# zeyadmohamedabdo/Visual-Question-Answering-VQA-system

Measured on AMD Instinct MI355X. Metric: image-question pairs/sec (train step), higher is better.
Workload: dtype bf16; 1 GPU; VQA train step fwd+CE+bwd+allreduce+clip+AdamW, batch 512/GPU, 3x224x224 images, 20 tokens, d=256, 4 text layers, 49 image tokens, 1000 answers, dropout on (BASELINE configs[2]); batch_per_gpu=512, global_batch=512, parallelism=dp1, reducer=off

## Files before the change

### include/vqa_hip.h

```cpp
#ifndef VQA_HIP_H
#define VQA_HIP_H
#include <stdint.h>
#ifdef __cplusplus
extern "C" {
#endif
typedef struct ihipStream_t* hipStream_t;

int vqa_igemm_mtiles(int M, int N, int loader);
int vqa_igemm_variant(int dtype, int loader, int M, int N, int Kw, int B, int H, int W, int C, int Ho, int Wo,
                      int R, int S, int stride, int pad);
int vqa_igemm(int dtype, int loader, const void* a, const void* w, void* out, const float* bias, const void* addend,
              const void* addmask, const void* outmask , float* stats, int M, int N, int Kw, int B, int H, int W, int C, int Ho, int Wo,
              int R, int S, int stride, int pad, int transposed, int relu, float drop_p, unsigned long long drop_seed,
              int stats_mode ,
              hipStream_t stream);
int vqa_linear_dgrad_act(int dtype, const void* dz, const void* wt, void* dx, const void* addend, const void* outact, float drop_p,
                         int M, int Kin, int N, hipStream_t stream);
int vqa_wgrad_plan(int dtype, int loader, int M, int N, int Kw, int B, int H, int W, int C, int R, int S, long long* ws_floats,
                   int* kind, int* tile_n, int* tile_k, int* nsplit);
int vqa_wgrad(int dtype, int loader, const void* dy, const void* x, float* dw, int M, int N, int Kw, int B, int H, int W,
              int C, int Ho, int Wo, int R, int S, int stride, int pad, float* ws, long long ws_floats, hipStream_t stream);
int vqa_pack_rows(int dtype, const float* in, void* out, int N, int K, int Kp, hipStream_t stream);
int vqa_pack_transpose(int dtype, const float* in, void* out, int N, int T, int C, int ldo, int col0, int flip, hipStream_t stream);
int vqa_pack_transpose_batch(int dtype, const float* flat, void* out, const long long* desc, int nd, int total_blocks, hipStream_t stream);
// ... 28 lines not shown
                        float* ws , long long ws_floats, hipStream_t stream);
int vqa_wgrad3x3_c128_blocks(int B, int H, int W);
int vqa_wgrad3x3_c128(const void* x, const void* dy, float* dw, int B, int H, int W, float* ws, long long ws_floats, hipStream_t stream);
int vqa_wgrad3x3_c64_blocks(int B, int H, int W);
int vqa_wgrad3x3_c64(const void* x, const void* dy, float* dw , int B, int H, int W,
                     float* ws ,
                     long long ws_floats, hipStream_t stream);
long long vqa_wgrad_group_ws(int dtype, int njobs, const int* M, const int* N, const int* Kw);
int vqa_wgrad_group(int dtype, int njobs, const void* const* dy, const void* const* x, float* const* dw, const int* M, const int* N,
                    const int* Kw, float* ws, long long ws_floats, hipStream_t stream);
int vqa_slab_reduce(const float* ws, float* dw, int nslabs, long long n, hipStream_t stream);
int vqa_dgrad_s2(int dtype, const void* dy, const void* dyd, const void* wt, void* out, int B, int H, int W, int C,
                 int Ho, int Wo, int N, int R, int pad, hipStream_t stream);
int vqa_stem_conv_blocks(int B, int H, int W);
int vqa_stem_pack(const float* w_krsc, void* wstem, hipStream_t stream);
int vqa_stem_conv(const float* img, const void* wstem, void* out, float* stats, int B, int H, int W, hipStream_t stream);
int vqa_stem_conv_pool_ok(int B, int H, int W);
int vqa_stem_conv_pool(const float* img, const void* wstem, const float* coef, void* out, int B, int H, int W, hipStream_t stream);
int vqa_stem_wgrad_blocks(int B, int H, int W);
int vqa_stem_wgrad(const float* img, const void* dy, float* dw , int B, int H, int W,
                   float* ws , long long ws_floats, hipStream_t stream);
int vqa_stem_wgrad_fused(const float* img, const void* y, const void* dpool, const uint8_t* idx, const float* coef,
                         const float* bcoef, float* dw, int B, int H, int W, float* ws, long long ws_floats, hipStream_t stream);
int vqa_stem_dgrad_pack(int dtype, const float* w_krsc, void* wpk, hipStream_t stream);
int vqa_stem_dgrad(int dtype, const void* dy, const void* wpk, float* dimg, int B, int H, int W, hipStream_t stream);
int vqa_stem_dgrad_fused_ok(int B, int H, int W);
int vqa_stem_dgrad_fused(const void* y, const void* dpool, const uint8_t* idx, const float* coef, const float* bcoef, const void* wpk,
                         float* dimg, int B, int H, int W, hipStream_t stream);

int vqa_bn_stats_finalize(const float* part, int tiles, int C, double count, const float* gamma, const float* beta,
                          float* running_mean, float* running_var, long long* num_batches_tracked, float momentum, float eps,
                          double* scratch , float* coef, hipStream_t stream);
int vqa_bn_eval_coef(int C, const float* gamma, const float* beta, const float* running_mean, const float* running_var,
                     float eps, float* coef, hipStream_t stream);
int vqa_bn_apply(int dtype, const void* y, const float* coef, const void* res, const float* rcoef, void* out,
                 long long numel, int C, int relu, hipStream_t stream);
int vqa_bn_apply_pool_chunks(int dtype, int HW, int C);
int vqa_bn_apply_pool(int dtype, const void* y, const float* coef, const void* res, const float* rcoef, void* out, int B, int HW, int C,
// ... 151 lines not shown
```

### visual-question-answering-vqa-system_amd/_lib.py

```python
from __future__ import annotations

import ctypes as C
import os

import torch

_HERE = os.path.dirname(os.path.abspath(__file__))
LIB_PATH = os.path.join(_HERE, "libvqa_hip.so")

P, I, F, D, LL, ULL = C.c_void_p, C.c_int, C.c_float, C.c_double, C.c_longlong, C.c_ulonglong

SIGNATURES = {
    "vqa_gemm8p": [P, P, P, I, I, I, P],
    "vqa_gemm4w": [P, P, P, I, I, I, P],
    "vqa_conv8p_ok": [I, I, I, I, I],
    "vqa_conv8p": [P, P, P, P, P, P, P, P, P, P, I, P, P, I, I, I, I, I, I, I, P],
    "vqa_igemm_mtiles": [I, I, I],
    "vqa_igemm_variant": [I] * 15,
    "vqa_igemm": [I, I, P, P, P, P, P, P, P, P] + [I] * 15 + [F, ULL, I, P],
    "vqa_linear_dgrad_act": [I, P, P, P, P, P, F, I, I, I, P],
    "vqa_wgrad_plan": [I] * 11 + [P, P, P, P, P],
    "vqa_wgrad": [I, I, P, P, P] + [I] * 13 + [P, LL, P],
    "vqa_pack_rows": [I, P, P, I, I, I, P],
    "vqa_pack_transpose": [I, P, P, I, I, I, I, I, I, P],
# ... 7 lines not shown
    "vqa_conv3x3_c64p_epi": [P, P, P, P, P, P, I, I, I, P],
    "vqa_conv3x3_c64p_bnred": [P, P, P, P, P, P, I, I, I, P],
    "vqa_conv3x3_c64p_bn": [P, P, P, P, P, P, P, P, P, P, P, I, I, I, I, D, F, F, P],
    "vqa_wgrad3x3_c64_bn_ok": [I, I, I],
    "vqa_wgrad3x3_c64_bn": [P, P, P, P, I, I, I, P, LL, P],
    "vqa_wgrad3x3_c128_blocks": [I, I, I],
    "vqa_wgrad3x3_c128": [P, P, P, I, I, I, P, LL, P],
    "vqa_wgrad3x3_c64_blocks": [I, I, I],
    "vqa_wgrad3x3_c64": [P, P, P, I, I, I, P, LL, P],
    "vqa_wgrad_group_ws": [I, I, P, P, P],
    "vqa_wgrad_group": [I, I, P, P, P, P, P, P, P, LL, P],
    "vqa_slab_reduce": [P, P, I, LL, P],
    "vqa_dgrad_s2": [I, P, P, P, P, I, I, I, I, I, I, I, I, I, P],
    "vqa_stem_conv_blocks": [I, I, I],
    "vqa_stem_pack": [P, P, P],
    "vqa_stem_conv": [P, P, P, P, I, I, I, P],
    "vqa_stem_conv_pool_ok": [I, I, I],
    "vqa_stem_conv_pool": [P, P, P, P, I, I, I, P],
    "vqa_stem_wgrad_blocks": [I, I, I],
    "vqa_stem_wgrad": [P, P, P, I, I, I, P, LL, P],
    "vqa_stem_wgrad_fused": [P, P, P, P, P, P, P, I, I, I, P, LL, P],
    "vqa_stem_dgrad_pack": [I, P, P, P],
    "vqa_stem_dgrad": [I, P, P, P, I, I, I, P],
    "vqa_stem_dgrad_fused_ok": [I, I, I],
    "vqa_stem_dgrad_fused": [P, P, P, P, P, P, P, I, I, I, P],
    "vqa_bn_stats_finalize": [P, I, I, D, P, P, P, P, P, F, F, P, P, P],
    "vqa_bn_eval_coef": [I, P, P, P, P, F, P, P],
    "vqa_bn_apply": [I, P, P, P, P, P, LL, I, I, P],
    "vqa_bn_apply_pool_chunks": [I, I, I],
    "vqa_bn_apply_pool": [I, P, P, P, P, P, I, I, I, I, P, P],
    "vqa_se_bwd_blocks": [I, I, I, I],
    "vqa_se_bwd_scratch": [I, I, I, I, I],
    "vqa_bn_bwd_blocks": [LL],
    "vqa_bn_bwd_reduce": [I, P, P, P, P, P, P, P, LL, I, I, I, P],
    "vqa_bn_acc_words": [I, I],
    "vqa_bn_apply_acc": [I, P, P, P, P, P, P, P, P, P, P, P, P, P, P, P, P, P, I, I, I, I, D, F, F, P, P],
# ... 45 lines not shown
    "vqa_answer_scores": [P, P, P, P, I, I, I, I, P, P],
    "vqa_cross_entropy_soft": [I, P, P, P, I, P, P, P, I, I, F, P, P, P, P, P],
    "vqa_challenge_accuracy_update": [P, P, P, I, P, I, I, P],
    "vqa_convert": [I, I, P, P, LL, P],
    "vqa_sumsq": [P, LL, P, P],
    "vqa_image_normalize": [P, P, P, I, I, I, F, F, F, F, F, F, P],
    "vqa_image_color_jitter": [P, P, P, I, I, I, P, P, F, F, F, F, F, F, P, P],
    "vqa_image_resize_ws": [I, P, P, I, I, I],
    "vqa_image_resize": [P, P, P, P, P, I, I, I, I, I, P, P, P, F, F, F, F, F, F, P, LL, P],
    "vqa_pack_tokens": [P, P, P, P, I, I, I, I, I, I, P],
    "vqa_adamw": [P, P, P, P, LL, F, F, F, F, F, LL, P, F, F, P, P, P, P],
    "vqa_sumsq_ranges": [P, P, I, LL, P, P],
    "vqa_adamw_ranges": [P, P, P, P, P, I, LL, F, F, F, F, F, LL, P, F, F, P, P, P, P, I, P, P],
}
_RET_LL = {"vqa_image_resize_ws", "vqa_wgrad_group_ws", "vqa_spatial_bwd_scratch", "vqa_se_bwd_scratch", "vqa_layernorm_bwd_ws", "vqa_bias_act_bwd_ws"}
_NO_STATUS = _RET_LL | {"vqa_wgrad3x3_c64_blocks", "vqa_bn_acc_words", "vqa_bn_apply_pool_chunks", "vqa_se_bwd_blocks", "vqa_wgrad3x3_c128_blocks", "vqa_layernorm_bwd_folds", "vqa_bias_act_bwd_fold_rows", "vqa_conv3x3_c64p_blocks", "vqa_stem_wgrad_blocks", "vqa_igemm_mtiles", "vqa_igemm_variant", "vqa_bn_bwd_blocks", "vqa_stem_conv_blocks", "vqa_stem_conv_pool_ok", "vqa_stem_dgrad_fused_ok", "vqa_wgrad3x3_c64_bn_ok", "vqa_conv8p_ok"}

_lib = None


def lib() -> C.CDLL:
    global _lib
    if _lib is None:
        if not os.path.exists(LIB_PATH):
            raise RuntimeError(f"{LIB_PATH} is missing: build it with __graft_entry__.build() "
                               "(hipcc --offload-arch=gfx950); there is no CPU fallback")
        L = C.CDLL(LIB_PATH)
        for name, args in SIGNATURES.items():
            fn = getattr(L, name)
            fn.argtypes = args
            fn.restype = LL if name in _RET_LL else I
# ... 39 lines not shown
```

### visual-question-answering-vqa-system_amd/csrc/stem_conv.hip

```cpp
#include <cstdlib>
#include "common.h"
#include <type_traits>
#include "stem_route.h"

namespace {
constexpr int RB = 4;
constexpr int PR = 2 * RB + 5;
constexpr int KP = 192;
constexpr int LDW = KP + 8;
constexpr int LDCS = 64 + 8;
}

template <int PROWS, int XO, int CH>
__device__ __forceinline__ void stem_fill_patch(bf16_t* __restrict__ patch, int PW, __amdgpu_buffer_rsrc_t rsImg, int b, int ih_base,
                                                int H, int W, int tid) {
  static_assert(XO & 1, "odd column offset");
  const int W4 = W >> 2, nitems = 3 * PROWS * W4, nh = PW - W;
  const float inv_w4 = 1.0f / (float)W4, inv_nh = 1.0f / (float)nh;
  for (int i = tid; i < 3 * PROWS * nh; i += 256) {
    const int row = (int)(((float)i + 0.5f) * inv_nh), k = i - row * nh;
    patch[row * PW + (k < XO ? k : W + k)] = 0;
  }
  for (int base = tid; base < nitems; base += 256 * CH) {
    f32x4 v[CH]; int dst[CH];
#pragma unroll
// ... 18 lines not shown
      d[3] = f2bf(v[i][3]);
    }
  }
}

__global__ void stem_pack_kernel(const float* __restrict__ w, bf16_t* __restrict__ out) {
  const int i = blockIdx.x * blockDim.x + threadIdx.x;
  if (i >= 64 * KP) return;
  const int n = i / KP, k = i - n * KP, pair = k >> 3, s = k & 7;
  float v = 0.f;
  if (pair < 21 && s < 7) { const int c = pair / 7, r = pair - c * 7; v = w[((n * 7 + r) * 7 + s) * 3 + c]; }
  out[i] = f2bf(v);
}

__global__ __launch_bounds__(256) void stem_conv_kernel(const float* __restrict__ img, const bf16_t* __restrict__ wst, bf16_t* __restrict__ out,
                                                        float* __restrict__ stats, int H, int W, int Ho, int Wo) {
  extern __shared__ __attribute__((aligned(16))) char smem[];
  const int PW = 2 * Wo + 8;
  bf16_t* patch = reinterpret_cast<bf16_t*>(smem);
  bf16_t* Wl = patch + 3 * PR * PW;
  bf16_t* Cst = Wl;
  float* red = reinterpret_cast<float*>(Wl + 64 * LDW);
  const int tid = threadIdx.x, lane = tid & 63, wave = tid >> 6, g = lane >> 4, li = lane & 15;
  const int rblocks = Ho / RB;
  const int b = blockIdx.x / rblocks, oh0 = (blockIdx.x - b * rblocks) * RB;

  for (int v = tid; v < 64 * (KP / 8); v += 256) {
    const int n = v / (KP / 8), kv = v - n * (KP / 8);
    *reinterpret_cast<u32x4*>(&Wl[n * LDW + kv * 8]) = *reinterpret_cast<const u32x4*>(&wst[n * KP + kv * 8]);
  }
  const int ih_base = 2 * oh0 - 3;
// ... 2 lines not shown
    const int iw = x - 3;
    const bool cok = iw >= 0 && iw < W;
    float vals[3 * PR];
#pragma unroll
    for (int row = 0; row < 3 * PR; ++row) {
      const int c = row / PR, pr = row - c * PR, ih = ih_base + pr;
      const bool ok = cok && ih >= 0 && ih < H;
      const int ihc = min(max(ih, 0), H - 1), iwc = min(max(iw, 0), W - 1);
      const float t = __builtin_bit_cast(float, __builtin_amdgcn_raw_buffer_load_b32(rsImg, (((b * 3 + c) * H + ihc) * W + iwc) * 4, 0, 0));
      vals[row] = ok ? t : 0.f;
    }
#pragma unroll
    for (int row = 0; row < 3 * PR; ++row) patch[row * PW + x] = f2bf(vals[row]);
  }
  __syncthreads();

  bf16x8 bfr[6][4];
#pragma unroll
  for (int kk = 0; kk < 6; ++kk)
#pragma unroll
    for (int nt = 0; nt < 4; ++nt)
      bfr[kk][nt] = *reinterpret_cast<const bf16x8*>(&Wl[(nt * 16 + li) * LDW + kk * 32 + g * 8]);
  __syncthreads();

  float ssum[4] = {0.f, 0.f, 0.f, 0.f}, ssq[4] = {0.f, 0.f, 0.f, 0.f};
  const int mtiles_row = Wo / 16, mtiles = RB * mtiles_row;
  bf16_t* mycs = Cst + wave * 16 * LDCS;
  for (int mt = wave; mt < mtiles; mt += 4) {
    const int orow = mt / mtiles_row, ow0 = (mt - orow * mtiles_row) * 16;
    f32x4 acc[4];
// ... 310 lines not shown
  for (int j = 0; j < 3; ++j) {
    const int k2 = wave * 48 + j * 16 + li, pair = k2 >> 3, s = k2 & 7;
    if (pair >= 21 || s >= 7) continue;
    const int c = pair / 7, r = pair - c * 7;
#pragma unroll
    for (int i = 0; i < 4; ++i)
#pragma unroll
      for (int rr = 0; rr < 4; ++rr) {
        const size_t o = (size_t)(i * 16 + g * 4 + rr) * 147 + (r * 7 + s) * 3 + c;
        if (ws) ws[(size_t)blockIdx.x * (64 * 147) + o] = acc[i][j][rr];
        else atomicAdd(dw + o, acc[i][j][rr]);
      }
  }
}

extern "C" int vqa_slab_reduce(const float* ws, float* dw, int nslabs, long long n, hipStream_t st);

static size_t stem_wgrad_shm(int Wo, int nsplit) {
  const int PW = 2 * Wo + 8, MP = (Wo / nsplit + 31) / 32 * 32;
  return (size_t)(3 * PRW * PW + MP * LDA + MP * LDD) * 2;
}
static int stem_nsplit(int Wo) {
  const int env = vqa_env_int("VQA_STEM_NSPLIT", 0);
  if (env > 0 && Wo % (8 * env) == 0) return env;
  const int floor_ = Wo > 64 ? 2 : 1;
  for (int n = floor_; n <= 16; ++n)
    if (Wo % (8 * n) == 0 && stem_wgrad_shm(Wo, n) <= (size_t)160 * 1024 / 3) return n;
  return floor_;
}
static int stem_wgrad_grid(int B, int Ho, int Wo, size_t* shm_out) {
  const size_t shm = stem_wgrad_shm(Wo, stem_nsplit(Wo));
  if (shm_out) *shm_out = shm;
  if (shm > 160 * 1024) return 0;
  const int nblocks = B * (Ho / RBW);
  const int cap = 256 * (int)((160 * 1024) / shm > 4 ? 4 : (160 * 1024) / shm);
  return nblocks < cap ? nblocks : cap;
}

extern "C" {

int vqa_stem_conv_blocks(int B, int H, int W) {
  const int Ho = (H + 6 - 7) / 2 + 1, Wo = (W + 6 - 7) / 2 + 1;
  if (Ho % RB || Wo % 16 || Wo > 256) return 0;
  return B * (Ho / RB);
}
int vqa_stem_pack(const float* w_krsc, void* wstem , hipStream_t st) {
  if (!w_krsc || !wstem) return VQA_EARG;
  hipLaunchKernelGGL(stem_pack_kernel, dim3((64 * KP + 255) / 256), dim3(256), 0, st, w_krsc, (bf16_t*)wstem);
  VQA_LAUNCH_CHECK(); return VQA_OK;
}
int vqa_stem_conv(const float* img, const void* wstem, void* out, float* stats, int B, int H, int W, hipStream_t st) {
  const int nb = vqa_stem_conv_blocks(B, H, W);
  if (!img || !wstem || !out || nb <= 0 || (size_t)B * 3 * H * W * 4 >= 0x7fffffffull) return VQA_EARG;
  const int Ho = (H + 6 - 7) / 2 + 1, Wo = (W + 6 - 7) / 2 + 1, PW = 2 * Wo + 8;
  const size_t shm = (size_t)(3 * PR * PW + 64 * LDW) * 2 + 4 * 64 * 2 * 4;
  (void)vqa_ensure_lds(reinterpret_cast<const void*>(&stem_conv_kernel), shm);
  hipLaunchKernelGGL(stem_conv_kernel, dim3(nb), dim3(256), shm, st, img, (const bf16_t*)wstem, (bf16_t*)out, stats, H, W, Ho, Wo);
  VQA_LAUNCH_CHECK(); return VQA_OK;
}

static size_t stem_conv_pool_shm(int H, int W, int* ctiles_out, int* pw_out) {
  const int Ho = (H + 6 - 7) / 2 + 1, Wo = (W + 6 - 7) / 2 + 1, Hp = (Ho + 2 - 3) / 2 + 1, Wp = (Wo + 2 - 3) / 2 + 1;
  if (H < 7 || W < 7 || (Ho & 1) || (Wo & 1) || Hp % PRB) return 0;
  const int ctiles = (Wp + 6) / 7;
  const int PW = (2 * (14 * ctiles + 2) + 8 + 7) / 8 * 8;
  if (ctiles_out) *ctiles_out = ctiles;
  if (pw_out) *pw_out = PW;
  const size_t shm = (size_t)(3 * PRP * PW + 64 * LDW) * 2;
  return shm <= 160 * 1024 ? shm : 0;
}
int vqa_stem_conv_pool_ok(int B, int H, int W) {
  return B > 0 && stem_conv_pool_shm(H, W, nullptr, nullptr) > 0 && (size_t)B * 3 * H * W * 4 < 0x7fffffffull;
// ... 41 lines not shown
  const int nsplit = stem_nsplit(Wo);
  const int PW = 2 * Wo + 8, MP = (Wo / nsplit + 31) / 32 * 32;
  const size_t shm = (size_t)(3 * PRW * PW + MP * LDA + MP * LDD) * 2;
  if (shm > 160 * 1024) return VQA_EARG;
  (void)vqa_ensure_lds(reinterpret_cast<const void*>(&stem_wgrad_kernel<true>), shm);
  int nblocks = B * (Ho / RBW);
  const int cap = 256 * (int)((160 * 1024) / shm > 4 ? 4 : (160 * 1024) / shm);
  int grid = nblocks < cap ? nblocks : cap;
  float* w = (ws && ws_floats >= (long long)grid * 64 * 147) ? ws : nullptr;
  hipLaunchKernelGGL(stem_wgrad_kernel<true>, dim3(grid), dim3(256), shm, st, img, (const bf16_t*)y, dw, B, H, W, Ho, Wo,
                     (const bf16_t*)dpool, idx, coef, bcoef, Hp, Wp, nsplit, w);
  VQA_LAUNCH_CHECK();
  return w ? vqa_slab_reduce(w, dw, grid, 64 * 147, st) : VQA_OK;
}

}
```

### visual-question-answering-vqa-system_amd/engine.py

```python
from __future__ import annotations

import math
from typing import Callable, Dict, List, Optional

import torch

from . import kernels as K
from . import layout as LY
from ._lib import call, dt, ptr


def _streams_overlap(a: "torch.cuda.Stream", b: "torch.cuda.Stream", cycles: int = 1_500_000) -> bool:
    ea, eb = torch.cuda.Event(), torch.cuda.Event()
    with torch.cuda.stream(a):
        torch.cuda._sleep(cycles)
        ea.record()
    with torch.cuda.stream(b):
        torch.cuda._sleep(1000)
        eb.record()
    eb.synchronize()
    ok = not ea.query()
    ea.synchronize()
    return ok

# ... 55 lines not shown
        self.fuse_bn1_reduce = True
        self.use_conv8p_bwd = True
        self._accbuf = None
        self._accpos = 0
        self._stem_fcoef = None
        self.fold_eval = True
        self._fold = None
        self.infer_precision = "bf16"
        self._foldmx = None
        self.stem_w = None
        self.side, self.side2 = pick_concurrent_streams(flat.device, 2) if flat.is_cuda else (None, None)
        self.two_streams = True
        self.capture = None
        self.capture_io = None
        self.fuse_stem_eval = True
        self.mark = None

    def P(self, name):
        e = self.E[name]
        return self.flat[e.offset: e.offset + e.numel]

    def Wm(self, name):
        return LY.mat_of(self.wsrc, self.E[name])

    def _packT(self, key, pieces, rows, ld):
        t = self._wt.get(key)
        if t is None:
            t = torch.empty((rows, ld), device=self.flat.device, dtype=self.dtype)
            for off, n, tt, c, col0, flip in pieces:
                K.pack_transpose(self.flat[off: off + n * tt * c].view(n, tt, c), self.dtype, out=t, ldo=ld, col0=col0, flip=flip)
# ... 369 lines not shown
        phead = cfg["answer_dropout"] if htrain else 0.0
        dev = images.device

        main = torch.cuda.current_stream()
        use_side = self.two_streams and self.side is not None
        if use_side:
            ev0 = torch.cuda.Event(); ev0.record(main)
        H1, W1 = (IH + 6 - 7) // 2 + 1, (IW + 6 - 7) // 2 + 1
        M = B * H1 * W1
        sgeom = (B, IH, IW, 3, H1, W1, 7, 7, 2, 3)
        Hp, Wp = (H1 + 2 - 3) // 2 + 1, (W1 + 2 - 3) // 2 + 1
        x = None
        if self.fuse_stem_eval and not training and not cnn_tape and self.stem_w2 is not None:
            x = K.stem_conv_pool(images, self.stem_w2, self._bn_coef("image_encoder.stem.1", None, 0, 64, M, False), B, IH, IW)
        if x is None:
            if self.stem_w2 is not None and K.stem_conv_blocks(B, IH, IW) > 0:
                y, st, mt = K.stem_conv(images, self.stem_w2, B, IH, IW, training)
            else:
                y, st, mt = K.igemm(images, self.stem_w, M, 64, self.stem_kp, sgeom, dtype=T, loader=K.LOADER_STEM, want_stats=training)
            coef = self._bn_coef("image_encoder.stem.1", st, mt, 64, M, training)
            x = torch.empty((B * Hp * Wp, 64), device=dev, dtype=T)
            idx = torch.empty((B * Hp * Wp, 64), device=dev, dtype=torch.uint8)
            call("vqa_stem_pool_fwd", dt(T), ptr(y), ptr(coef), ptr(x), ptr(idx), B, H1, W1, 64)
            if cnn_tape:
                tape["stem"] = dict(images=images, y=y, coef=coef, idx=idx, geom=sgeom, H1=H1, W1=W1)
        H, W, C = Hp, Wp, 64
        d, heads = cfg["embed_dim"], cfg["num_attention_heads"]
        hd = d // heads
        Bt, L = token_ids.shape
        rows = Bt * L
        pe = self.buf["text_encoder.positional_encoding.pe"]
        if L > pe.shape[1]:
            raise RuntimeError(f"sequence length {L} exceeds max_question_length {pe.shape[1]}")
        text = {}

        def issue_text():
            if use_side:
                self.side.wait_event(ev0)
            with torch.cuda.stream(self.side if use_side else main):
                emb_e = self.E["text_encoder.token_embedding.weight"]
# ... 908 lines not shown
        bc = torch.empty((3, 64), device=dxc.device, dtype=torch.float32)
        bnp = "image_encoder.stem.1"
        call("vqa_bn_bwd_finalize", ptr(slab), nb, 64, 1, float(B * H1 * W1), ptr(self.P(bnp + ".weight")), ptr(st["coef"]),
             int(training), ptr(self._gslice(G, bnp + ".weight")), ptr(self._gslice(G, bnp + ".bias")), ptr(bc))
        if after_reduce is not None:
            after_reduce()
        wpk = K.stem_dgrad_pack(self.P("image_encoder.stem.0.weight"), T) if want_dimg else None
        dimg = None
        skip_w = self._frozen_g(self._gslice(G, "image_encoder.stem.0.weight"))
        if fused and skip_w:
            pass
        elif fused:
            dwv = self._gslice(G, "image_encoder.stem.0.weight")
            e0 = K.prof_begin()
            ws, wsf = K.stem_wgrad_scratch(dxc.device, B, IH, IW)
            call("vqa_stem_wgrad_fused", ptr(st["images"]), ptr(st["y"]), ptr(dxc), ptr(st["idx"]), ptr(st["coef"]), ptr(bc), ptr(dwv), B, IH, IW,
                 ptr(ws), wsf)
            if e0 is not None:
                K.prof_end(e0, "stem_wgrad_kernel<true>", 2.0 * B * H1 * W1 * 64 * 147,
                           B * 3 * IH * IW * 4 + B * H1 * W1 * 64 * 2 + dxc.numel() * 3)
        if fused:
            if want_dimg:
                if K.stem_dgrad_fused_ok(B, IH, IW):
                    dimg = K.stem_dgrad_fused(st["y"], dxc, st["idx"], st["coef"], bc, wpk, B, IH, IW)
                else:
                    dy = torch.empty_like(st["y"])
                    call("vqa_stem_bwd_apply", dt(T), ptr(dxc), ptr(st["idx"]), ptr(st["y"]), ptr(st["coef"]), ptr(bc), ptr(dy), B, H1, W1, 64)
                    dimg = K.stem_dgrad(dy, wpk, B, IH, IW)
        else:
            dy = torch.empty_like(st["y"])
            call("vqa_stem_bwd_apply", dt(T), ptr(dxc), ptr(st["idx"]), ptr(st["y"]), ptr(st["coef"]), ptr(bc), ptr(dy), B, H1, W1, 64)
            if not skip_w:
                K.wgrad(dy, st["images"], LY.mat_of(G, self.E["image_encoder.stem.0.weight"]), B * H1 * W1, 64, 147, st["geom"], dtype=T,
                        loader=K.LOADER_STEM)
            if want_dimg:
# ... 86 lines not shown
```

### visual-question-answering-vqa-system_amd/kernels.py

```python
from __future__ import annotations

import os

import torch

from . import _lib as L
from ._lib import call, dt, ptr

LOADER_NHWC, LOADER_STEM = 0, 1

PROFILE = None
PROFILE_VARIANTS = []
PROFILE_STAGED = {}


def prof_begin():
    if PROFILE is None:
        return None
    e0 = torch.cuda.Event(enable_timing=True)
    e0.record()
    return e0


def prof_end(e0, sym, flops, nbytes):
# ... 270 lines not shown

def stem_dgrad_fused(y, dpool, idx, coef, bc, wpk, B, H, W):
    dimg = torch.empty((B, 3, H, W), device=y.device, dtype=torch.float32)
    Ho, Wo, flops = _stem_dgrad_cost(B, H, W)
    e0 = prof_begin()
    call("vqa_stem_dgrad_fused", ptr(y), ptr(dpool), ptr(idx), ptr(coef), ptr(bc), ptr(wpk), ptr(dimg), B, H, W)
    if e0 is not None:
        prof_end(e0, "stem_dgrad_kernel<bf16,true>", flops, B * Ho * Wo * 64 * 2 + dpool.numel() * 3 + dimg.numel() * 4)
    return dimg


def stem_conv_blocks(B, H, W) -> int:
    return L.count("vqa_stem_conv_blocks", B, H, W)


def stem_conv(img, wstem, B, H, W, want_stats):
    nb = stem_conv_blocks(B, H, W)
    Ho, Wo = (H + 6 - 7) // 2 + 1, (W + 6 - 7) // 2 + 1
    y = torch.empty((B * Ho * Wo, 64), device=img.device, dtype=torch.bfloat16)
    stats = torch.empty((nb, 2, 64), device=img.device, dtype=torch.float32) if want_stats else None
    e0 = prof_begin()
    call("vqa_stem_conv", ptr(img), ptr(wstem), ptr(y), ptr(stats), B, H, W)
    if e0 is not None:
        prof_end(e0, "stem_conv_kernel", 2.0 * B * Ho * Wo * 64 * 147, B * 3 * H * W * 4 + B * Ho * Wo * 64 * 2)
    return y, stats, nb


def stem_conv_pool(img, wstem, coef, B, H, W):
    if not L.count("vqa_stem_conv_pool_ok", B, H, W):
        return None
    Ho, Wo = (H + 6 - 7) // 2 + 1, (W + 6 - 7) // 2 + 1
    Hp, Wp = (Ho + 2 - 3) // 2 + 1, (Wo + 2 - 3) // 2 + 1
    x = torch.empty((B * Hp * Wp, 64), device=img.device, dtype=torch.bfloat16)
    e0 = prof_begin()
    call("vqa_stem_conv_pool", ptr(img), ptr(wstem), ptr(coef), ptr(x), B, H, W)
    if e0 is not None:
        prof_end(e0, "stem_conv_pool_kernel", 2.0 * B * Ho * Wo * 64 * 147, B * 3 * H * W * 4 + B * Hp * Wp * 64 * 2)
    return x

# ... 262 lines not shown
```

### visual-question-answering-vqa-system_amd/layout.py

```python
from __future__ import annotations

import math
from dataclasses import dataclass
from typing import Dict, List, Tuple

import torch

STAGE_CHANNELS = (64, 128, 256, 512)
ALIGN = 8

CONFIG_KEYS = ("vocab_size", "embed_dim", "num_answers", "use_se_attention", "use_spatial_attention", "se_reduction",
               "num_transformer_layers", "num_attention_heads", "ffn_hidden_dim", "max_question_length",
               "num_cross_layers", "use_gating", "dropout", "answer_dropout")


@dataclass
class Entry:
    name: str
    shape: Tuple[int, ...]
    kind: str
    is_param: bool
    offset: int = -1
    krsc: bool = False

# ... 140 lines not shown
def bucket_ranges(entries: List[Entry]) -> List[Tuple[str, int, int]]:
    groups = ["answer_head.", "fusion.", "text_encoder.", "image_encoder.stage4.", "image_encoder.stage3.",
              "image_encoder.stage2.", "image_encoder.stage1.", "image_encoder.stem."]
    out = []
    total = flat_size(entries)
    params = [e for e in entries if e.is_param]
    for g in groups:
        es = [e for e in params if e.name.startswith(g)]
        if not es:
            continue
        lo = es[0].offset
        nxt = [e.offset for e in params if e.offset > es[-1].offset]
        hi = min(nxt) if nxt else total
        out.append((g.rstrip("."), lo, hi))
    return out
```

Before: 41930 pairs/s.

## Emit space-to-depth bf16 image copy in stem conv for wgrad reuse

```diff
diff --git a/include/vqa_hip.h b/include/vqa_hip.h
--- a/include/vqa_hip.h
+++ b/include/vqa_hip.h
@@ -66,7 +66,8 @@
                  int Ho, int Wo, int N, int R, int pad, hipStream_t stream);
 int vqa_stem_conv_blocks(int B, int H, int W);
 int vqa_stem_pack(const float* w_krsc, void* wstem, hipStream_t stream);
-int vqa_stem_conv(const float* img, const void* wstem, void* out, float* stats, int B, int H, int W, hipStream_t stream);
+int vqa_stem_conv(const float* img, const void* wstem, void* out, float* stats, void* s2d ,
+                  int B, int H, int W, hipStream_t stream);
 int vqa_stem_conv_pool_ok(int B, int H, int W);
 int vqa_stem_conv_pool(const float* img, const void* wstem, const float* coef, void* out, int B, int H, int W, hipStream_t stream);
 int vqa_stem_wgrad_blocks(int B, int H, int W);
@@ -74,6 +75,10 @@
                    float* ws , long long ws_floats, hipStream_t stream);
 int vqa_stem_wgrad_fused(const float* img, const void* y, const void* dpool, const uint8_t* idx, const float* coef,
                          const float* bcoef, float* dw, int B, int H, int W, float* ws, long long ws_floats, hipStream_t stream);
+int vqa_stem_s2d_ok(int B, int H, int W);
+int vqa_stem_wgrad_s2d(const void* s2d, const void* dy, float* dw, int B, int H, int W, float* ws, long long ws_floats, hipStream_t stream);
+int vqa_stem_wgrad_s2d_fused(const void* s2d, const void* y, const void* dpool, const uint8_t* idx, const float* coef,
+                             const float* bcoef, float* dw, int B, int H, int W, float* ws, long long ws_floats, hipStream_t stream);
 int vqa_stem_dgrad_pack(int dtype, const float* w_krsc, void* wpk, hipStream_t stream);
 int vqa_stem_dgrad(int dtype, const void* dy, const void* wpk, float* dimg, int B, int H, int W, hipStream_t stream);
 int vqa_stem_dgrad_fused_ok(int B, int H, int W);
diff --git a/visual-question-answering-vqa-system_amd/_lib.py b/visual-question-answering-vqa-system_amd/_lib.py
--- a/visual-question-answering-vqa-system_amd/_lib.py
+++ b/visual-question-answering-vqa-system_amd/_lib.py
@@ -45,12 +45,15 @@
     "vqa_dgrad_s2": [I, P, P, P, P, I, I, I, I, I, I, I, I, I, P],
     "vqa_stem_conv_blocks": [I, I, I],
     "vqa_stem_pack": [P, P, P],
-    "vqa_stem_conv": [P, P, P, P, I, I, I, P],
+    "vqa_stem_conv": [P, P, P, P, P, I, I, I, P],
     "vqa_stem_conv_pool_ok": [I, I, I],
     "vqa_stem_conv_pool": [P, P, P, P, I, I, I, P],
     "vqa_stem_wgrad_blocks": [I, I, I],
     "vqa_stem_wgrad": [P, P, P, I, I, I, P, LL, P],
     "vqa_stem_wgrad_fused": [P, P, P, P, P, P, P, I, I, I, P, LL, P],
+    "vqa_stem_s2d_ok": [I, I, I],
+    "vqa_stem_wgrad_s2d": [P, P, P, I, I, I, P, LL, P],
+    "vqa_stem_wgrad_s2d_fused": [P, P, P, P, P, P, P, I, I, I, P, LL, P],
     "vqa_stem_dgrad_pack": [I, P, P, P],
     "vqa_stem_dgrad": [I, P, P, P, I, I, I, P],
     "vqa_stem_dgrad_fused_ok": [I, I, I],
@@ -126,7 +129,7 @@
     "vqa_adamw_ranges": [P, P, P, P, P, I, LL, F, F, F, F, F, LL, P, F, F, P, P, P, P, I, P, P],
 }
 _RET_LL = {"vqa_image_resize_ws", "vqa_wgrad_group_ws", "vqa_spatial_bwd_scratch", "vqa_se_bwd_scratch", "vqa_layernorm_bwd_ws", "vqa_bias_act_bwd_ws"}
-_NO_STATUS = _RET_LL | {"vqa_wgrad3x3_c64_blocks", "vqa_bn_acc_words", "vqa_bn_apply_pool_chunks", "vqa_se_bwd_blocks", "vqa_wgrad3x3_c128_blocks", "vqa_layernorm_bwd_folds", "vqa_bias_act_bwd_fold_rows", "vqa_conv3x3_c64p_blocks", "vqa_stem_wgrad_blocks", "vqa_igemm_mtiles", "vqa_igemm_variant", "vqa_bn_bwd_blocks", "vqa_stem_conv_blocks", "vqa_stem_conv_pool_ok", "vqa_stem_dgrad_fused_ok", "vqa_wgrad3x3_c64_bn_ok", "vqa_conv8p_ok"}
+_NO_STATUS = _RET_LL | {"vqa_wgrad3x3_c64_blocks", "vqa_bn_acc_words", "vqa_bn_apply_pool_chunks", "vqa_se_bwd_blocks", "vqa_wgrad3x3_c128_blocks", "vqa_layernorm_bwd_folds", "vqa_bias_act_bwd_fold_rows", "vqa_conv3x3_c64p_blocks", "vqa_stem_wgrad_blocks", "vqa_igemm_mtiles", "vqa_igemm_variant", "vqa_bn_bwd_blocks", "vqa_stem_conv_blocks", "vqa_stem_conv_pool_ok", "vqa_stem_dgrad_fused_ok", "vqa_stem_s2d_ok", "vqa_wgrad3x3_c64_bn_ok", "vqa_conv8p_ok"}
 
 _lib = None
 
diff --git a/visual-question-answering-vqa-system_amd/csrc/stem_conv.hip b/visual-question-answering-vqa-system_amd/csrc/stem_conv.hip
--- a/visual-question-answering-vqa-system_amd/csrc/stem_conv.hip
+++ b/visual-question-answering-vqa-system_amd/csrc/stem_conv.hip
@@ -9,6 +9,7 @@
 constexpr int KP = 192;
 constexpr int LDW = KP + 8;
 constexpr int LDCS = 64 + 8;
+typedef __attribute__((ext_vector_type(2))) uint32_t u32x2;
 }
 
 template <int PROWS, int XO, int CH>
@@ -57,7 +58,7 @@
 }
 
 __global__ __launch_bounds__(256) void stem_conv_kernel(const float* __restrict__ img, const bf16_t* __restrict__ wst, bf16_t* __restrict__ out,
-                                                        float* __restrict__ stats, int H, int W, int Ho, int Wo) {
+                                                        float* __restrict__ stats, bf16_t* __restrict__ s2d, int H, int W, int Ho, int Wo) {
   extern __shared__ __attribute__((aligned(16))) char smem[];
   const int PW = 2 * Wo + 8;
   bf16_t* patch = reinterpret_cast<bf16_t*>(smem);
@@ -90,6 +91,38 @@
     for (int row = 0; row < 3 * PR; ++row) patch[row * PW + x] = f2bf(vals[row]);
   }
   __syncthreads();
+
+  if (s2d) {
+    const int XC = PW >> 1, upr = XC >> 1;
+    const int nrows = RB + (oh0 + RB == Ho ? 2 : 0);
+    for (int u = tid; u < nrows * upr; u += 256) {
+      const int yr = u / upr, ux = u - yr * upr;
+      uint16_t e[2][3][4];
+#pragma unroll
+      for (int py = 0; py < 2; ++py)
+#pragma unroll
+        for (int c = 0; c < 3; ++c) {
+          const u32x2 t = *reinterpret_cast<const u32x2*>(&patch[(c * PR + 2 * yr + py) * PW + 4 * ux]);
+          e[py][c][0] = (uint16_t)t[0]; e[py][c][1] = (uint16_t)(t[0] >> 16);
+          e[py][c][2] = (uint16_t)t[1]; e[py][c][3] = (uint16_t)(t[1] >> 16);
+        }
+      uint32_t o[12];
+#pragma unroll
+      for (int i = 0; i < 12; ++i) {
+        uint32_t h[2];
+#pragma unroll
+        for (int k = 0; k < 2; ++k) {
+          const int el = 2 * i + k, cell = el / 12, rem = el - cell * 12, py = rem / 6, px = (rem - py * 6) / 3, c = rem % 3;
+          h[k] = e[py][c][2 * cell + px];
+        }
+        o[i] = h[0] | (h[1] << 16);
+      }
+      u32x4* d = reinterpret_cast<u32x4*>(s2d + (((size_t)b * (Ho + 3) + oh0 + yr) * XC + 2 * ux) * 12);
+      d[0] = u32x4{o[0], o[1], o[2], o[3]};
+      d[1] = u32x4{o[4], o[5], o[6], o[7]};
+      d[2] = u32x4{o[8], o[9], o[10], o[11]};
+    }
+  }
 
   bf16x8 bfr[6][4];
 #pragma unroll
@@ -430,6 +463,142 @@
   }
 }
 
+namespace {
+constexpr int SROWS = RBW + 3;
+constexpr int CELL = 12;
+constexpr int ZROW = 48;
+}
+template <bool FUSED>
+__global__ __launch_bounds__(256) void stem_wgrad_s2d_kernel(const bf16_t* __restrict__ s2d, const bf16_t* __restrict__ dy, float* __restrict__ dw,
+                                                             int B, int Ho, int Wo, const bf16_t* __restrict__ dpool,
+                                                             const uint8_t* __restrict__ idx, const float* __restrict__ coef,
+                                                             const float* __restrict__ bc, int Hp, int Wp, int nsplit, float* __restrict__ ws) {
+  extern __shared__ __attribute__((aligned(16))) char smem[];
+  const int XC = Wo + 4;
+  const int Wh = Wo / nsplit;
+  const int MP = (Wh + 31) / 32 * 32;
+  bf16_t* patch = reinterpret_cast<bf16_t*>(smem);
+  bf16_t* zrow = patch + SROWS * XC * CELL;
+  bf16_t* Dy = zrow + ZROW;
+  const int tid = threadIdx.x, lane = tid & 63, wave = tid >> 6, g = lane >> 4, li = lane & 15;
+  const int q = li >> 2, pp = li & 3;
+  for (int i = tid; i < ZROW; i += 256) zrow[i] = 0;
+  for (int i = tid; i < (MP - Wh) * LDD; i += 256) Dy[Wh * LDD + i] = 0;
+
+  float f_sc[8], f_sh[8], f_a[8], f_b[8], f_c[8];
+  if (FUSED) {
+    const int c0f = (tid & 7) * 8;
+#pragma unroll
+    for (int j = 0; j < 8; ++j) {
+      f_sc[j] = coef[c0f + j]; f_sh[j] = coef[64 + c0f + j];
+      f_a[j] = bc[c0f + j]; f_b[j] = bc[64 + c0f + j]; f_c[j] = bc[128 + c0f + j];
+    }
+  }
+  const __amdgpu_buffer_rsrc_t rsP = __builtin_amdgcn_make_buffer_rsrc(const_cast<bf16_t*>(FUSED ? dpool : dy), 0, FUSED ? B * Hp * Wp * 64 * 2 : 0, 0x00020000);
+  const __amdgpu_buffer_rsrc_t rsI = __builtin_amdgcn_make_buffer_rsrc(const_cast<uint8_t*>(FUSED ? idx : reinterpret_cast<const uint8_t*>(dy)), 0, FUSED ? B * Hp * Wp * 64 : 0, 0x00020000);
+  const __amdgpu_buffer_rsrc_t rsS = __builtin_amdgcn_make_buffer_rsrc(const_cast<bf16_t*>(s2d), 0, B * (Ho + 3) * XC * CELL * 2, 0x00020000);
+  const __amdgpu_buffer_rsrc_t rsDy = __builtin_amdgcn_make_buffer_rsrc(const_cast<bf16_t*>(dy), 0, B * Ho * Wo * 64 * 2, 0x00020000);
+  f32x4 acc[4][3];
+#pragma unroll
+  for (int i = 0; i < 4; ++i)
+#pragma unroll
+    for (int j = 0; j < 3; ++j) acc[i][j] = f32x4{0.f, 0.f, 0.f, 0.f};
+
+  const int rblocks = Ho / RBW, nblocks = B * rblocks;
+  const int npieces = SROWS * XC * CELL / 8;
+  for (int blk = blockIdx.x; blk < nblocks; blk += gridDim.x) {
+    const int b = blk / rblocks, oh0 = (blk - b * rblocks) * RBW;
+    __syncthreads();
+    const int sbase = ((b * (Ho + 3) + oh0) * XC) * CELL * 2;
+    for (int base = tid; base < npieces; base += 256 * 4) {
+      u32x4 v[4];
+#pragma unroll
+      for (int i = 0; i < 4; ++i)
+        v[i] = __builtin_bit_cast(u32x4, __builtin_amdgcn_raw_buffer_load_b128(rsS, sbase + (base + 256 * i) * 16, 0, 0));
+#pragma unroll
+      for (int i = 0; i < 4; ++i)
+        if (base + 256 * i < npieces) *reinterpret_cast<u32x4*>(patch + (base + 256 * i) * 8) = v[i];
+    }
+    for (int unit = 0; unit < RBW * nsplit; ++unit) {
+      const int orow = unit / nsplit, px0 = (unit - orow * nsplit) * Wh;
+      __syncthreads();
+      const int dyr_b = (((b * Ho + oh0 + orow) * Wo + px0) * 64) * 2;
+      if constexpr (FUSED) {
+        auto stage_row = [&](auto odd) {
+          for (int v = tid; v < (Wh >> 1) * 8; v += 256) {
+            const int pq = v >> 3, cv = v & 7;
+            Vec16<bf16_t> yy[2];
+            yy[0].raw = __builtin_bit_cast(u32x4, __builtin_amdgcn_raw_buffer_load_b128(rsDy, dyr_b + (2 * pq) * 128 + cv * 16, 0, 0));
+            yy[1].raw = __builtin_bit_cast(u32x4, __builtin_amdgcn_raw_buffer_load_b128(rsDy, dyr_b + (2 * pq + 1) * 128 + cv * 16, 0, 0));
+            float g8[2][8];
+            stem_route_pair_buf<decltype(odd)::value>(rsP, rsI, yy, f_sc, f_sh, b, oh0 + orow, (px0 >> 1) + pq, cv * 8, Hp, Wp, g8);
+#pragma unroll
+            for (int q2 = 0; q2 < 2; ++q2) {
+              Vec16<bf16_t> o;
+#pragma unroll
+              for (int j = 0; j < 8; ++j) o.set(j, f_a[j] * g8[q2][j] + f_b[j] * yy[q2].get(j) + f_c[j]);
+              uint32_t* d = reinterpret_cast<uint32_t*>(&Dy[(2 * pq + q2) * LDD + cv * 8]);
+              d[0] = o.raw[0]; d[1] = o.raw[1]; d[2] = o.raw[2]; d[3] = o.raw[3];
+            }
+          }
+        };
+        if ((oh0 + orow) & 1) stage_row(std::true_type{});
+        else stage_row(std::false_type{});
+      } else {
+        for (int v = tid; v < Wh * 8; v += 256) {
+          const int px = v >> 3, cv = v & 7;
+          const u32x4 val = __builtin_bit_cast(u32x4, __builtin_amdgcn_raw_buffer_load_b128(rsDy, dyr_b + v * 16, 0, 0));
+          uint32_t* d = reinterpret_cast<uint32_t*>(&Dy[px * LDD + cv * 8]);
+          d[0] = val[0]; d[1] = val[1]; d[2] = val[2]; d[3] = val[3];
+        }
+      }
+      __syncthreads();
+      typedef __attribute__((ext_vector_type(8))) short i16x8;
+      const bf16_t* xrow = patch + ((orow + wave) * XC + px0) * CELL + 4 * pp;
+      for (int ks = 0; ks < MP / 32; ++ks) {
+        const int p = ks * 32 + 8 * g + q;
+        const bf16_t* yb = Dy + p * LDD + 4 * pp;
+        const bf16_t* xlo = p < Wh ? xrow + p * CELL : zrow + 4 * pp;
+        const bf16_t* xhi = p < Wh ? xlo + 4 * CELL : xlo;
+        bf16x8 af[4], bfv[3];
+#pragma unroll
+        for (int i = 0; i < 4; ++i) {
+          i16x4 lo = __builtin_amdgcn_ds_read_tr16_b64_v4i16((i16x4 __attribute__((address_space(3)))*)(yb + i * 16));
+          i16x4 hi = __builtin_amdgcn_ds_read_tr16_b64_v4i16((i16x4 __attribute__((address_space(3)))*)(yb + 4 * LDD + i * 16));
+          i16x8 t = {lo[0], lo[1], lo[2], lo[3], hi[0], hi[1], hi[2], hi[3]};
+          af[i] = __builtin_bit_cast(bf16x8, t);
+        }
+#pragma unroll
+        for (int j = 0; j < 3; ++j) {
+          i16x4 lo = __builtin_amdgcn_ds_read_tr16_b64_v4i16((i16x4 __attribute__((address_space(3)))*)(xlo + j * 16));
+          i16x4 hi = __builtin_amdgcn_ds_read_tr16_b64_v4i16((i16x4 __attribute__((address_space(3)))*)(xhi + j * 16));
+          i16x8 t = {lo[0], lo[1], lo[2], lo[3], hi[0], hi[1], hi[2], hi[3]};
+          bfv[j] = __builtin_bit_cast(bf16x8, t);
+        }
+#pragma unroll
+        for (int i = 0; i < 4; ++i)
+#pragma unroll
+          for (int j = 0; j < 3; ++j)
+            acc[i][j] = __builtin_amdgcn_mfma_f32_16x16x32_bf16(af[i], bfv[j], acc[i][j], 0, 0, 0);
+      }
+    }
+  }
+#pragma unroll
+  for (int j = 0; j < 3; ++j) {
+    const int k = j * 16 + li, sp = k / CELL, rem = k - sp * CELL, py = rem / 6, px = (rem - py * 6) / 3, c = rem % 3;
+    const int r = 2 * wave + py, s = 2 * sp + px;
+    if (r >= 7 || s >= 7) continue;
+#pragma unroll
+    for (int i = 0; i < 4; ++i)
+#pragma unroll
+      for (int rr = 0; rr < 4; ++rr) {
+        const size_t o = (size_t)(i * 16 + g * 4 + rr) * 147 + (r * 7 + s) * 3 + c;
+        if (ws) ws[(size_t)blockIdx.x * (64 * 147) + o] = acc[i][j][rr];
+        else atomicAdd(dw + o, acc[i][j][rr]);
+      }
+  }
+}
+
 extern "C" int vqa_slab_reduce(const float* ws, float* dw, int nslabs, long long n, hipStream_t st);
 
 static size_t stem_wgrad_shm(int Wo, int nsplit) {
@@ -453,6 +622,17 @@
   return nblocks < cap ? nblocks : cap;
 }
 
+static size_t stem_wgrad_s2d_shm(int Wo, int nsplit) {
+  const int MP = (Wo / nsplit + 31) / 32 * 32;
+  return (size_t)(SROWS * (Wo + 4) * CELL + ZROW + MP * LDD) * 2;
+}
+static bool stem_s2d_shape_ok(int B, int H, int W) {
+  const int Ho = (H + 6 - 7) / 2 + 1, Wo = (W + 6 - 7) / 2 + 1;
+  if (B <= 0 || H < 7 || W < 7 || Ho % RBW || Wo % 16 || Wo > 256) return false;
+  return (size_t)B * (Ho + 3) * (Wo + 4) * CELL * 2 < 0x7fff0000ull && (size_t)B * Ho * Wo * 64 * 2 < 0x7fffffffull &&
+         (size_t)B * 3 * H * W * 4 < 0x7fffffffull;
+}
+
 extern "C" {
 
 int vqa_stem_conv_blocks(int B, int H, int W) {
@@ -465,13 +645,14 @@
   hipLaunchKernelGGL(stem_pack_kernel, dim3((64 * KP + 255) / 256), dim3(256), 0, st, w_krsc, (bf16_t*)wstem);
   VQA_LAUNCH_CHECK(); return VQA_OK;
 }
-int vqa_stem_conv(const float* img, const void* wstem, void* out, float* stats, int B, int H, int W, hipStream_t st) {
+int vqa_stem_conv(const float* img, const void* wstem, void* out, float* stats, void* s2d, int B, int H, int W, hipStream_t st) {
   const int nb = vqa_stem_conv_blocks(B, H, W);
+  if (s2d && !stem_s2d_shape_ok(B, H, W)) return VQA_EARG;
   if (!img || !wstem || !out || nb <= 0 || (size_t)B * 3 * H * W * 4 >= 0x7fffffffull) return VQA_EARG;
   const int Ho = (H + 6 - 7) / 2 + 1, Wo = (W + 6 - 7) / 2 + 1, PW = 2 * Wo + 8;
   const size_t shm = (size_t)(3 * PR * PW + 64 * LDW) * 2 + 4 * 64 * 2 * 4;
   (void)vqa_ensure_lds(reinterpret_cast<const void*>(&stem_conv_kernel), shm);
-  hipLaunchKernelGGL(stem_conv_kernel, dim3(nb), dim3(256), shm, st, img, (const bf16_t*)wstem, (bf16_t*)out, stats, H, W, Ho, Wo);
+  hipLaunchKernelGGL(stem_conv_kernel, dim3(nb), dim3(256), shm, st, img, (const bf16_t*)wstem, (bf16_t*)out, stats, (bf16_t*)s2d, H, W, Ho, Wo);
   VQA_LAUNCH_CHECK(); return VQA_OK;
 }
 
@@ -543,4 +724,36 @@
   return w ? vqa_slab_reduce(w, dw, grid, 64 * 147, st) : VQA_OK;
 }
 
-}
+int vqa_stem_s2d_ok(int B, int H, int W) { return stem_s2d_shape_ok(B, H, W) ? 1 : 0; }
+
+static int stem_wgrad_s2d_launch(bool fused, const void* s2d, const void* y, const void* dpool, const uint8_t* idx, const float* coef,
+                                 const float* bcoef, float* dw, int B, int H, int W, float* ws, long long ws_floats, hipStream_t st) {
+  if (!s2d || !y || !dw || !stem_s2d_shape_ok(B, H, W)) return VQA_EARG;
+  if (fused && (!dpool || !idx || !coef || !bcoef)) return VQA_EARG;
+  const int Ho = (H + 6 - 7) / 2 + 1, Wo = (W + 6 - 7) / 2 + 1, Hp = (Ho + 2 - 3) / 2 + 1, Wp = (Wo + 2 - 3) / 2 + 1;
+  const int nsplit = stem_nsplit(Wo);
+  const int grid = stem_wgrad_grid(B, Ho, Wo, nullptr);
+  const size_t shm = stem_wgrad_s2d_shm(Wo, nsplit);
+  if (grid <= 0 || shm > 160 * 1024) return VQA_EARG;
+  float* w = (ws && ws_floats >= (long long)grid * 64 * 147) ? ws : nullptr;
+  if (fused) {
+    (void)vqa_ensure_lds(reinterpret_cast<const void*>(&stem_wgrad_s2d_kernel<true>), shm);
+    hipLaunchKernelGGL(stem_wgrad_s2d_kernel<true>, dim3(grid), dim3(256), shm, st, (const bf16_t*)s2d, (const bf16_t*)y, dw, B, Ho, Wo,
+                       (const bf16_t*)dpool, idx, coef, bcoef, Hp, Wp, nsplit, w);
+  } else {
+    (void)vqa_ensure_lds(reinterpret_cast<const void*>(&stem_wgrad_s2d_kernel<false>), shm);
+    hipLaunchKernelGGL(stem_wgrad_s2d_kernel<false>, dim3(grid), dim3(256), shm, st, (const bf16_t*)s2d, (const bf16_t*)y, dw, B, Ho, Wo,
+                       (const bf16_t*)nullptr, (const uint8_t*)nullptr, (const float*)nullptr, (const float*)nullptr, 0, 0, nsplit, w);
+  }
+  VQA_LAUNCH_CHECK();
+  return w ? vqa_slab_reduce(w, dw, grid, 64 * 147, st) : VQA_OK;
+}
+int vqa_stem_wgrad_s2d(const void* s2d, const void* dy, float* dw, int B, int H, int W, float* ws, long long ws_floats, hipStream_t st) {
+  return stem_wgrad_s2d_launch(false, s2d, dy, nullptr, nullptr, nullptr, nullptr, dw, B, H, W, ws, ws_floats, st);
+}
+int vqa_stem_wgrad_s2d_fused(const void* s2d, const void* y, const void* dpool, const uint8_t* idx, const float* coef, const float* bcoef,
+                             float* dw, int B, int H, int W, float* ws, long long ws_floats, hipStream_t st) {
+  return stem_wgrad_s2d_launch(true, s2d, y, dpool, idx, coef, bcoef, dw, B, H, W, ws, ws_floats, st);
+}
+
+}
diff --git a/visual-question-answering-vqa-system_amd/engine.py b/visual-question-answering-vqa-system_amd/engine.py
--- a/visual-question-answering-vqa-system_amd/engine.py
+++ b/visual-question-answering-vqa-system_amd/engine.py
@@ -93,6 +93,8 @@
         self.capture = None
         self.capture_io = None
         self.fuse_stem_eval = True
+        self.stem_s2d = True
+        self._s2d_buf, self._s2d_gen = None, 0
         self.mark = None
 
     def P(self, name):
@@ -492,8 +494,16 @@
         if self.fuse_stem_eval and not training and not cnn_tape and self.stem_w2 is not None:
             x = K.stem_conv_pool(images, self.stem_w2, self._bn_coef("image_encoder.stem.1", None, 0, 64, M, False), B, IH, IW)
         if x is None:
+            s2d = None
             if self.stem_w2 is not None and K.stem_conv_blocks(B, IH, IW) > 0:
-                y, st, mt = K.stem_conv(images, self.stem_w2, B, IH, IW, training)
+                if self.stem_s2d and cnn_tape and K.stem_s2d_ok(B, IH, IW):
+                    we = self.E["image_encoder.stem.0.weight"]
+                    if plan is None or not plan.frozen(we.offset, we.numel):
+                        if self._s2d_buf is None or tuple(self._s2d_buf.shape) != LY.stem_s2d_shape(B, IH, IW):
+                            self._s2d_buf = K.stem_s2d_alloc(dev, B, IH, IW)
+                        self._s2d_gen += 1
+                        s2d = (self._s2d_buf, self._s2d_gen)
+                y, st, mt = K.stem_conv(images, self.stem_w2, B, IH, IW, training, s2d=None if s2d is None else s2d[0])
             else:
                 y, st, mt = K.igemm(images, self.stem_w, M, 64, self.stem_kp, sgeom, dtype=T, loader=K.LOADER_STEM, want_stats=training)
             coef = self._bn_coef("image_encoder.stem.1", st, mt, 64, M, training)
@@ -501,7 +511,7 @@
             idx = torch.empty((B * Hp * Wp, 64), device=dev, dtype=torch.uint8)
             call("vqa_stem_pool_fwd", dt(T), ptr(y), ptr(coef), ptr(x), ptr(idx), B, H1, W1, 64)
             if cnn_tape:
-                tape["stem"] = dict(images=images, y=y, coef=coef, idx=idx, geom=sgeom, H1=H1, W1=W1)
+                tape["stem"] = dict(images=images, y=y, coef=coef, idx=idx, geom=sgeom, H1=H1, W1=W1, s2d=s2d)
         H, W, C = Hp, Wp, 64
         d, heads = cfg["embed_dim"], cfg["num_attention_heads"]
         hd = d // heads
@@ -1440,11 +1450,19 @@
             dwv = self._gslice(G, "image_encoder.stem.0.weight")
             e0 = K.prof_begin()
             ws, wsf = K.stem_wgrad_scratch(dxc.device, B, IH, IW)
-            call("vqa_stem_wgrad_fused", ptr(st["images"]), ptr(st["y"]), ptr(dxc), ptr(st["idx"]), ptr(st["coef"]), ptr(bc), ptr(dwv), B, IH, IW,
-                 ptr(ws), wsf)
-            if e0 is not None:
-                K.prof_end(e0, "stem_wgrad_kernel<true>", 2.0 * B * H1 * W1 * 64 * 147,
-                           B * 3 * IH * IW * 4 + B * H1 * W1 * 64 * 2 + dxc.numel() * 3)
+            s2d = st.get("s2d")
+            if self.stem_s2d and s2d is not None and (s2d[0] is not self._s2d_buf or s2d[1] == self._s2d_gen):
+                call("vqa_stem_wgrad_s2d_fused", ptr(s2d[0]), ptr(st["y"]), ptr(dxc), ptr(st["idx"]), ptr(st["coef"]), ptr(bc), ptr(dwv),
+                     B, IH, IW, ptr(ws), wsf)
+                if e0 is not None:
+                    K.prof_end(e0, "stem_wgrad_kernel<true>", 2.0 * B * H1 * W1 * 64 * 147,
+                               s2d[0].numel() * 2 * 7 // 4 + B * H1 * W1 * 64 * 2 + dxc.numel() * 3)
+            else:
+                call("vqa_stem_wgrad_fused", ptr(st["images"]), ptr(st["y"]), ptr(dxc), ptr(st["idx"]), ptr(st["coef"]), ptr(bc), ptr(dwv),
+                     B, IH, IW, ptr(ws), wsf)
+                if e0 is not None:
+                    K.prof_end(e0, "stem_wgrad_kernel<true>", 2.0 * B * H1 * W1 * 64 * 147,
+                               B * 3 * IH * IW * 4 + B * H1 * W1 * 64 * 2 + dxc.numel() * 3)
         if fused:
             if want_dimg:
                 if K.stem_dgrad_fused_ok(B, IH, IW):
diff --git a/visual-question-answering-vqa-system_amd/kernels.py b/visual-question-answering-vqa-system_amd/kernels.py
--- a/visual-question-answering-vqa-system_amd/kernels.py
+++ b/visual-question-answering-vqa-system_amd/kernels.py
@@ -308,15 +308,25 @@
     return L.count("vqa_stem_conv_blocks", B, H, W)
 
 
-def stem_conv(img, wstem, B, H, W, want_stats):
+def stem_s2d_ok(B, H, W) -> bool:
+    return L.count("vqa_stem_s2d_ok", B, H, W) > 0
+
+
+def stem_s2d_alloc(device, B, H, W):
+    from . import layout as LY
+    return torch.zeros(LY.stem_s2d_shape(B, H, W), device=device, dtype=torch.bfloat16)
+
+
+def stem_conv(img, wstem, B, H, W, want_stats, s2d=None):
     nb = stem_conv_blocks(B, H, W)
     Ho, Wo = (H + 6 - 7) // 2 + 1, (W + 6 - 7) // 2 + 1
     y = torch.empty((B * Ho * Wo, 64), device=img.device, dtype=torch.bfloat16)
     stats = torch.empty((nb, 2, 64), device=img.device, dtype=torch.float32) if want_stats else None
     e0 = prof_begin()
-    call("vqa_stem_conv", ptr(img), ptr(wstem), ptr(y), ptr(stats), B, H, W)
-    if e0 is not None:
-        prof_end(e0, "stem_conv_kernel", 2.0 * B * Ho * Wo * 64 * 147, B * 3 * H * W * 4 + B * Ho * Wo * 64 * 2)
+    call("vqa_stem_conv", ptr(img), ptr(wstem), ptr(y), ptr(stats), ptr(s2d), B, H, W)
+    if e0 is not None:
+        prof_end(e0, "stem_conv_kernel", 2.0 * B * Ho * Wo * 64 * 147,
+                 B * 3 * H * W * 4 + B * Ho * Wo * 64 * 2 + (s2d.numel() * 2 if s2d is not None else 0))
     return y, stats, nb
 
 
diff --git a/visual-question-answering-vqa-system_amd/layout.py b/visual-question-answering-vqa-system_amd/layout.py
--- a/visual-question-answering-vqa-system_amd/layout.py
+++ b/visual-question-answering-vqa-system_amd/layout.py
@@ -178,3 +178,37 @@
         hi = min(nxt) if nxt else total
         out.append((g.rstrip("."), lo, hi))
     return out
+
+
+def stem_s2d_shape(B: int, H: int, W: int) -> Tuple[int, ...]:
+    Ho, Wo = (H + 6 - 7) // 2 + 1, (W + 6 - 7) // 2 + 1
+    return (B, Ho + 3, (Wo + 3 + 1) // 2 * 2, 2, 2, 3)
+
+
+def stem_s2d(img: torch.Tensor) -> torch.Tensor:
+    B, C, H, W = img.shape
+    _, YC, XC, _, _, _ = stem_s2d_shape(B, H, W)
+    pad = torch.zeros((B, C, 2 * YC, 2 * XC), dtype=img.dtype, device=img.device)
+    pad[:, :, 3:3 + H, 3:3 + W] = img
+    return pad.view(B, C, YC, 2, XC, 2).permute(0, 2, 4, 3, 5, 1).contiguous()
+
+
+def stem_s2d_kmap() -> List[Tuple[int, int, int, int, int, int, int, int]]:
+    out = []
+    for rp in range(4):
+        for sp in range(4):
+            for py in range(2):
+                for px in range(2):
+                    for c in range(3):
+                        r, s_ = 2 * rp + py, 2 * sp + px
+                        out.append((rp, sp, py, px, c, r, s_, int(r < 7 and s_ < 7)))
+    return out
+
+
+def stem_s2d_im2col(S: torch.Tensor, Ho: int, Wo: int) -> torch.Tensor:
+    B = S.shape[0]
+    out = torch.zeros((B, Ho, Wo, 7, 7, 3), dtype=S.dtype, device=S.device)
+    for rp, sp, py, px, c, r, s_, valid in stem_s2d_kmap():
+        if valid:
+            out[:, :, :, r, s_, c] = S[:, rp:rp + Ho, sp:sp + Wo, py, px, c]
+    return out.view(B, Ho, Wo, 147)
```

Measured after the change: 42340 pairs/s, median of 6. About the same (+1.0%).
